# sbokov/AddingDisparityFiltering

Hardware: AMD Instinct MI355X
Metric: filtered Mpixels/s (+ achieved HBM GB/s) on 4K disparity, 1/2/4/8 GPUs vs CPU ref (higher is better)
Workload: dtype f32

## Files before the change

### addingdisparityfiltering_amd/_lib.py

```python
import ctypes as C
import os

_HERE = os.path.dirname(os.path.abspath(__file__))
LIB_PATH = os.environ.get("ADF_WLS_LIB") or os.path.join(_HERE, "libadf_wls.so")

ADF_OK, ADF_EBADARG, ADF_ESIZE, ADF_EHIP, ADF_ENOMEM, ADF_ENODEV = range(6)
SOLVER_EXACT, SOLVER_WAVE = 0, 1
PATH_CONF_BAND, PATH_FUSED_FIRST_PASS, PATH_MERGED_PREP, PATH_SCALED_FUSED, PATH_SCALED_HALF = 1, 2, 4, 8, 16
PATH_ROW_WEIGHTS_GUIDE = 32
HANDOFF_PAIR_PLANE, HANDOFF_IMAGE, HANDOFF_IMAGE_PAIR_TAIL = 0, 1, 2
DEPTH_8U, DEPTH_16S, DEPTH_32S, DEPTH_32F = 0, 3, 4, 5
SGBM_COST_BT, SGBM_COST_CENSUS_DENSE, SGBM_COST_CENSUS_SPARSE = 0, 1, 2
BM_COST_SAD, BM_COST_CENSUS_DENSE, BM_COST_CENSUS_SPARSE = 0, 1, 2
SGBM_COST_MCT_DENSE, SGBM_COST_MCT_SPARSE, SGBM_COST_CENSUS_CS = 4, 5, 6
BM_COST_MCT_DENSE, BM_COST_MCT_SPARSE, BM_COST_CENSUS_CS = 4, 5, 6
SGBM_RIGHT_MATCHER, SGBM_RIGHT_FROM_VOLUME = 0, 1
MISSING_NONE, MISSING_MIN, MISSING_VALUE = 0, 1, 2
WMF_EXP, WMF_IV1, WMF_IV2, WMF_COS, WMF_JAC, WMF_OFF = range(6)
WMF_WEIGHT_ONE, WMF_TABLE_LEVELS, WMF_MAX_RADIUS = 65536, 3 * 256 * 256, 31
GF_MAX_RADIUS = 31
DTF_NC, DTF_IC, DTF_RF, DT_MAX_ITERS = 0, 1, 2, 8
DT_NC_MAX_RADIUS = 127
JBF_MAX_RADIUS = 31
BORDER_REPLICATE, BORDER_REFLECT, BORDER_WRAP, BORDER_REFLECT_101 = 1, 2, 3, 4
# ... 52 lines not shown
    ("adf_wls_set_lambda", _i, [_vp, _d]),
    ("adf_wls_get_lambda", _i, [_vp, C.POINTER(_d)]),
    ("adf_wls_set_sigma_color", _i, [_vp, _d]),
    ("adf_wls_get_sigma_color", _i, [_vp, C.POINTER(_d)]),
    ("adf_wls_set_lrc_thresh", _i, [_vp, _i]),
    ("adf_wls_get_lrc_thresh", _i, [_vp, C.POINTER(_i)]),
    ("adf_wls_set_depth_discontinuity_radius", _i, [_vp, _i]),
    ("adf_wls_get_depth_discontinuity_radius", _i, [_vp, C.POINTER(_i)]),
    ("adf_wls_set_fgs_params", _i, [_vp, _d, _i]),
    ("adf_wls_set_solver", _i, [_vp, _i]),
    ("adf_wls_get_solver", _i, [_vp, C.POINTER(_i)]),
    ("adf_wls_get_last_solver", _i, [_vp, C.POINTER(_i)]),
    ("adf_wls_get_last_path", _i, [_vp, C.POINTER(_i)]),
    ("adf_wls_get_last_solver_path", _i, [_vp, C.POINTER(_i)]),
    ("adf_wls_get_last_handoff", _i, [_vp, C.POINTER(_i)]),
    ("adf_wls_filter_device", _i, _FILTER_DEV),
    ("adf_wls_filter_host", _i, _FILTER_DEV[:-1]),
    ("adf_wls_filter_scaled_device", _i, _FILTER_SCALED_DEV),
    ("adf_wls_filter_scaled_host", _i, _FILTER_SCALED_DEV[:-1]),
    ("adf_wls_filter_f32_device", _i, _FILTER_DEV),
    ("adf_wls_filter_f32_host", _i, _FILTER_DEV[:-1]),
    ("adf_wls_filter_scaled_f32_device", _i, _FILTER_SCALED_DEV),
    ("adf_wls_filter_scaled_f32_host", _i, _FILTER_SCALED_DEV[:-1]),
    ("adf_wls_filter_typed_device", _i, _FILTER_TYPED_DEV),
    ("adf_wls_filter_typed_host", _i, _FILTER_TYPED_DEV[:-1]),
    ("adf_wls_get_confidence_device", _i, [_vp, _i, _vp, _pd, _vp]),
    ("adf_wls_get_confidence_host", _i, [_vp, _i, _vp, _pd]),
    ("adf_wls_get_device", _i, [_vp, C.POINTER(_i)]),
    ("adf_wls_get_roi", _i, [_vp, C.POINTER(Rect)]),
    ("adf_wls_sync", _i, [_vp, _vp]),
# ... 124 lines not shown
```

### addingdisparityfiltering_amd/csrc/adf_api.hip

```cpp
#include "adf_host.h"

#include <cmath>
#include <cstdio>
#include <cstdlib>
#include <cstring>
#include <new>

using namespace adf;

static inline int round_up(int v, int m) { return (v + m - 1) / m * m; }
template <class T> static const T* pairs_on(const T* p, ptrdiff_t pair_stride, int k)
{
    return p ? (const T*)((const char*)p + (ptrdiff_t)k * pair_stride) : nullptr;
}

static Geom make_geom(int W, int H, int rx, int ry, int rw, int rh)
{
    Geom g;
    g.W = W; g.H = H; g.rx = rx; g.ry = ry; g.rw = rw; g.rh = rh;
    g.pw = round_up(rw, 64);
    g.ph = round_up(rh, 64);
    size_t a = (size_t)round_up(rh, TILE_ROWS) * g.pw, b = (size_t)rw * g.ph;
    g.plane = ((a > b ? a : b) + 63) / 64 * 64;
    g.frame = (size_t)W * H;
// ... 67 lines not shown
    int epilogue; void* out; ptrdiff_t stride, pair_stride; int x0, y0, cn, c;
};

static double epilogue_bytes(int epilogue)
{
    return (epilogue == EPI_F32 || epilogue == EPI_WLS_CONF_F32) ? 4.0 : epilogue == EPI_U8 ? 1.0 : 2.0;
}

template <class Args>
static void set_final_out(Args& a, const FinalOut& fo)
{
    a.out = fo.out; a.out_stride = fo.stride; a.out_pair_stride = fo.pair_stride;
    a.out_x0 = fo.x0; a.out_y0 = fo.y0; a.out_cn = fo.cn; a.out_c = fo.c;
}

static int run_passes(bool wave, const Geom& g, const SolvePlanes& p, int n_rhs, float lambda, float atten, int num_iter,
                      const FinalOut& fo, int n_pairs, hipStream_t st, Profiler* prof = nullptr,
                      const FusedInputs* fuse = nullptr, const GuideWeights* gw = nullptr, float* image = nullptr, int image_m = 0)
{
    const double px = (double)g.rw * g.rh * n_pairs;
    float lam = lambda;
    for (int it = 0; it < num_iter; it++, lam *= atten) {
        const bool fused = it == 0 && fuse, last = it == num_iter - 1;
        const int epi = last ? fo.epilogue : EPI_PLANES;
        const double lo_b = (fused && fuse->lo_conf) ? 6.0 * fuse->lo_scale_x * fuse->lo_scale_y : (fused && fuse->dl_f32) ? 8.0 : 6.0;
        const double wb = gw ? (double)gw->ch : 4.0;
        const double hb = fused ? (wb + lo_b + 8.0) * px : (wb + 8.0 * n_rhs) * px;
        const double out_b = (last ? epilogue_bytes(fo.epilogue) : 4.0 * n_rhs) * px;
        const double vb = (4.0 + 4.0 * n_rhs) * px + out_b;
        if (wave) {
            WavePassArgs h{}, v{};
            h.C = p.CH; h.U0 = p.A0; h.U1 = p.A1;
            h.nscan = g.rh; h.len = g.rw; h.pitch = g.pw; h.plane = g.plane; h.lambda = lam;
            if (fused) h.fuse = *fuse;
            if (gw) h.gw = *gw;
            v.C = p.CV; v.U0 = p.A0; v.U1 = p.A1;
            v.nscan = g.rw; v.len = g.rh; v.pitch = g.pw; v.plane = g.plane; v.lambda = lam;
            if (last) set_final_out(v, fo);
            if (image && last && it > 0) {
                h.image = v.image = image; h.image_m = v.image_m = image_m;
                h.image_plane = v.image_plane = wave_image_floats(g.pw, image_m);
            }
            {
                ProfScope ps(prof, fused ? K_PASS_H_FIRST : K_PASS_H, hb, hb, st);
                HIP_TRY(launch_wave_hpass(h, n_rhs, n_pairs, st));
            }
            ProfScope ps(prof, last ? K_PASS_V_LAST : K_PASS_V, vb, vb, st);
            HIP_TRY(launch_wave_vpass(v, n_rhs, epi, n_pairs, st));
        } else {
            PassArgs h{}, v{};
            h.C = p.CH; h.U0 = p.A0; h.U1 = p.A1; h.D = p.D; h.F0 = p.F0; h.F1 = p.F1; h.O0 = p.B0; h.O1 = p.B1;
            h.nscan = g.rh; h.len = g.rw; h.pitch_in = g.ph; h.pitch_out = g.pw; h.plane = g.plane; h.lambda = lam;
            v.C = p.CV; v.U0 = p.B0; v.U1 = p.B1; v.D = p.D; v.F0 = p.F0; v.F1 = p.F1; v.O0 = p.A0; v.O1 = p.A1;
            v.nscan = g.rw; v.len = g.rh; v.pitch_in = g.pw; v.pitch_out = g.ph; v.plane = g.plane; v.lambda = lam;
            if (last) set_final_out(v, fo);
            {
// ... 44 lines not shown
    DevBuf stage;
    DevBuf scaled;
    size_t ws_limit = (size_t)64 << 30;
    Profiler prof;
    long long ws_sig[8] = {0, 0, 0, 0, 0, 0, 0, 0};
    hipStream_t side = nullptr;
    hipEvent_t ev_fork = nullptr, ev_join = nullptr;
    bool overlap = true;
    struct LazyConf { bool pending = false; ConfResize resize{}; } lazy_conf;
    bool scaled_half = true;
    bool scaled_fuse = true;
    bool conf_band = true;
    bool merge_small = true;
    bool row_weights_guide = true;
    bool handoff_image = true;
    long long handoff_min_px = HANDOFF_IMAGE_MIN_PX;
    int last_handoff = ADF_HANDOFF_PAIR_PLANE;
    static bool null_caller_of(hipStream_t s) { return s == nullptr || s == hipStreamLegacy || s == hipStreamPerThread; }
    int ensure_side(hipStream_t caller)
    {
        if (side) return ADF_OK;
        int least = 0, greatest = 0, prio = 0, cp = 0;
        if (hipDeviceGetStreamPriorityRange(&least, &greatest) != hipSuccess) { least = greatest = 0; (void)hipGetLastError(); }
        if (null_caller_of(caller) || stream_is_capturing(caller) || hipStreamGetPriority(caller, &cp) != hipSuccess) { cp = 0; (void)hipGetLastError(); }
        prio = (cp != greatest) ? greatest : (greatest < least ? greatest + 1 : greatest);
        if (null_caller_of(caller)) HIP_TRY(hipStreamCreateWithFlags(&side, hipStreamNonBlocking));
        else HIP_TRY(hipStreamCreateWithPriority(&side, hipStreamNonBlocking, prio));
        HIP_TRY(hipEventCreateWithFlags(&ev_fork, hipEventDisableTiming));
        HIP_TRY(hipEventCreateWithFlags(&ev_join, hipEventDisableTiming));
        return ADF_OK;
    }
};
// ... 10 lines not shown
    if (!h) return fail(ADF_ENOMEM, "adf_wls_create: out of host memory");
    if (hipGetDevice(&h->device) != hipSuccess) { delete h; return fail(ADF_EHIP, "hipGetDevice failed"); }
    h->use_confidence = use_confidence != 0;
    h->left_offset = l; h->right_offset = r; h->top_offset = t; h->bottom_offset = b;
    h->min_disp = 0; (void)min_disp;
    if (const char* e = getenv("ADF_WS_LIMIT_GB")) {
        double gb = atof(e);
        if (gb > 0) h->ws_limit = (size_t)(gb * (double)((size_t)1 << 30));
    }
    if (const char* e = getenv("ADF_NO_OVERLAP")) h->overlap = atoi(e) == 0;
    if (const char* e = getenv("ADF_CONF_BAND")) h->conf_band = atoi(e) != 0;
    if (const char* e = getenv("ADF_SCALED_FUSE")) h->scaled_fuse = atoi(e) != 0;
    if (const char* e = getenv("ADF_ROW_WEIGHTS_GUIDE")) h->row_weights_guide = atoi(e) != 0;
    if (const char* e = getenv("ADF_LO_HALF")) h->scaled_half = atoi(e) != 0;
    if (const char* e = getenv("ADF_LAST_HANDOFF_IMAGE")) h->handoff_image = atoi(e) != 0;
    if (const char* e = getenv("ADF_LAST_HANDOFF_MIN_PX")) h->handoff_min_px = atoll(e);
    if (const char* e = getenv("ADF_MERGE_SMALL")) h->merge_small = atoi(e) != 0;
    *out = h;
    return ADF_OK;
}

extern "C" void adf_wls_destroy(adf_wls_t* h)
{
    if (!h) return;
    DeviceScope ds(h->device);
    h->lut.release(); h->ws.release(); h->conf.release(); h->stage.release(); h->scaled.release();
    h->prof.destroy();
    if (h->ev_fork) hipEventDestroy(h->ev_fork);
    if (h->ev_join) hipEventDestroy(h->ev_join);
    if (h->side) hipStreamDestroy(h->side);
// ... 18 lines not shown
    return ADF_OK;
}

extern "C" int adf_wls_set_solver(adf_wls_t* h, int solver)
{
    NEED_HANDLE(h);
    if (solver != ADF_SOLVER_EXACT && solver != ADF_SOLVER_WAVE) return fail(ADF_EBADARG, "unknown solver %d", solver);
    h->solver = solver;
    return ADF_OK;
}
extern "C" int adf_wls_get_solver(const adf_wls_t* h, int* v) { NEED_HANDLE(h); if (v) *v = h->solver; return ADF_OK; }
extern "C" int adf_wls_get_last_solver(const adf_wls_t* h, int* v) { NEED_HANDLE(h); if (v) *v = h->last_solver; return ADF_OK; }
extern "C" int adf_wls_get_last_path(const adf_wls_t* h, int* v) { NEED_HANDLE(h); if (v) *v = h->last_path; return ADF_OK; }
extern "C" int adf_wls_get_last_solver_path(const adf_wls_t* h, int* v) { NEED_HANDLE(h); if (v) *v = h->last_solver_path; return ADF_OK; }
extern "C" int adf_wls_get_last_handoff(const adf_wls_t* h, int* v) { NEED_HANDLE(h); if (v) *v = h->last_handoff; return ADF_OK; }

extern "C" int adf_wls_get_device(const adf_wls_t* h, int* device) { NEED_HANDLE(h); if (device) *device = h->device; return ADF_OK; }
extern "C" int adf_wls_get_roi(const adf_wls_t* h, adf_rect* roi) { NEED_HANDLE(h); if (roi) *roi = h->roi; return ADF_OK; }
extern "C" size_t adf_wls_workspace_bytes(const adf_wls_t* h)
{
    return h ? h->ws.bytes + h->conf.bytes + h->stage.bytes + h->scaled.bytes + h->lut.bytes() : 0;
}

extern "C" int adf_wls_sync(adf_wls_t* h, void* stream)
{
    NEED_HANDLE(h);
    DeviceScope ds(h->device);
    HIP_TRY(hipStreamSynchronize((hipStream_t)stream));
    return ADF_OK;
}
// ... 293 lines not shown
        HIP_TRY(launch_conf_left(ca, n, st));
        return ADF_OK;
    }
    const double fill = o.fill ? fill_bytes(F - P, false, o.fill->out_f32 ? 4.0 : 2.0).alg : 0.0;
    ProfScope ps(prof, K_LRC, lrc_bytes(F, P, o.U0 != nullptr, m.rhs_f32() ? 4.0 : 2.0, fill), st);
    HIP_TRY(launch_lrc_prologue(lrc_args(m, o, g, r), n, st));
    return ADF_OK;
}

struct ChunkPlan {
    ConfStage stage;
    bool fork_weights;
    bool outside_on_side;
    bool guide_rows;
    bool image;
};

struct WlsPlan {
    Geom g;
    bool wave;
    RhsSource rhs;
    bool band;
    bool quant_planes;
    Geom glo; bool lo_band; size_t dhi_bytes;
    size_t per_pair; int chunk;
    int image_m;
    bool image_in_chor;
    ChunkPlan full, tail;
    int path;
    int solver_path;
    bool fused_first() const { return rhs == RHS_FUSED_VIEW || rhs == RHS_FUSED_LO; }
};

static ChunkPlan plan_chunk(const adf_wls* h, ConfStage stage, bool wave, bool guide_rows, bool image)
{
    const bool fork = stage != CONF_NONE && stage != CONF_MERGED && h->overlap;
    return ChunkPlan{stage, fork, fork && wave && stage != CONF_TWO_KERNEL, guide_rows && stage != CONF_MERGED, image};
}

static GuideWeights guide_weights(const adf_wls* h, const uint8_t* guide, const View& v, const Geom& g)
{
    return GuideWeights{guide, v.stride, v.pair_stride, v.ch, g.rx, g.ry, h->lut.cur};
}

static WlsPlan plan_wls(const adf_wls* h, const WlsCall& c)
{
    WlsPlan p{};
    const bool conf = h->use_confidence, f32in = c.dm.f32;
    const View& v = c.view;
    const Geom g = p.g = make_geom(v.W, v.H, c.rhi.x, c.rhi.y, c.rhi.width, c.rhi.height);
    p.wave = h->solver == ADF_SOLVER_WAVE && wave_fits(g);
    MapSource m = caller_maps(c.dm);
// ... 29 lines not shown
    const int image_m = (conf && p.wave && h->handoff_image && h->num_iter >= 2 && wave_hpass_image_fits(g.rw)) ? wave_vpass_image_m(g.rh) : 0;
    const long long roi_px = (long long)g.rw * g.rh;
    const bool may_merge = p.band && h->merge_small && prep_small_fits(g, h->disc_radius, v.ch, 1) && prep_small_guide_fits(g, v.stride, v.ch);
    auto chunk_for = [&](int im) {
        p.image_m = im;
        p.image_in_chor = im && guide_rows && !may_merge;
        p.per_pair = wls_pair_ws_bytes(g, conf, p.wave, !p.band, p.quant_planes, im, p.image_in_chor);
        p.chunk = (int)(h->ws_limit / p.per_pair);
        if (p.chunk < 1) p.chunk = 1;
        if (p.chunk > c.n_pairs) p.chunk = c.n_pairs;
    };
    chunk_for(image_m);
    if (image_m && roi_px * p.chunk < h->handoff_min_px) chunk_for(0);
    auto chunk_of = [&](int n) {
        const bool merged = p.band && h->merge_small && prep_small_fits(g, h->disc_radius, v.ch, n) && prep_small_guide_fits(g, v.stride, v.ch);
        return plan_chunk(h, merged ? CONF_MERGED : stage, p.wave, guide_rows, p.image_m && roi_px * n >= h->handoff_min_px);
    };
    p.full = chunk_of(p.chunk);
    p.tail = chunk_of(c.n_pairs % p.chunk ? c.n_pairs % p.chunk : p.chunk);
    p.path = ((p.band || p.lo_band) ? ADF_PATH_CONF_BAND : 0) |
             (p.fused_first() ? ADF_PATH_FUSED_FIRST_PASS : 0) |
             ((p.full.stage == CONF_MERGED || p.tail.stage == CONF_MERGED) ? ADF_PATH_MERGED_PREP : 0);
    p.solver_path = (p.full.guide_rows || p.tail.guide_rows) ? ADF_PATH_ROW_WEIGHTS_GUIDE : 0;
    if (p.rhs == RHS_FUSED_LO)
        p.path |= ADF_PATH_SCALED_FUSED |
                  (wave_hpass_lo_half(first_pass_probe(lo_fuse(h, c, p.lo_band, UNALLOCATED, m, nullptr, g), g.rw)) ? ADF_PATH_SCALED_HALF : 0);
    return p;
}

struct ScaledBufs { char* dhi; float *cl, *cr, *clo; float* taps; };

static int scaled_buffers(adf_wls_t* h, const WlsCall& c, const WlsPlan& plan, hipStream_t st, ScaledBufs& b, MapSource& lo)
// ... 43 lines not shown
    const bool conf = h->use_confidence, wave = plan.wave;
    const Geom& g = plan.g;
    const View& vw = c.view;
    const OutMap& om = c.om;
    const adf_rect& roi = c.rhi;
    const int n_pairs = c.n_pairs, W = vw.W, H = vw.H, gch = vw.ch;
    const double ob_px = (double)om.esz(), db_px = (double)c.dm.esz();
    Profiler* prof = &h->prof;
    int rc;
    ScaledBufs sb{};
    MapSource lo{};
    if (c.scaled && (rc = scaled_buffers(h, c, plan, st, sb, lo))) return rc;
    h->roi = roi; h->last_W = W; h->last_H = H; h->last_pairs = n_pairs;
    h->last_cpitch = g.cpitch; h->last_cx0 = g.cx0; h->last_path = 0; h->last_solver_path = 0;
    h->last_solver = wave ? ADF_SOLVER_WAVE : ADF_SOLVER_EXACT;
    h->last_handoff = ADF_HANDOFF_PAIR_PLANE;
    if ((rc = h->ws.reserve(plan.per_pair * (size_t)plan.chunk, st, FILL_ZERO))) return rc;
    if (conf && !c.scaled && (rc = ensure_conf_planes(h, g, n_pairs, st))) return rc;
    {
        const long long sig[8] = {W, H, roi.x, roi.y, roi.width, roi.height,
                                  (long long)plan.image_in_chor * 1024 + (long long)plan.image_m * 16 + (long long)plan.quant_planes * 8 + (long long)plan.band * 4 + (long long)wave * 2 + conf, plan.chunk};
        if (memcmp(sig, h->ws_sig, sizeof(sig)) != 0) {
            HIP_TRY(hipMemsetAsync(h->ws.p, 0, h->ws.bytes, st));
            memcpy(h->ws_sig, sig, sizeof(sig));
        }
    }
    float* base = (float*)h->ws.p;
    auto take = [&](size_t elems) { float* p = base; base += elems * (size_t)plan.chunk; return p; };
    SolvePlanes p{};
    p.CH = take(g.plane);
    float* const image_rest = plan.image_in_chor ? take(wave_image_floats(g.pw, plan.image_m) - g.plane) : nullptr;
// ... 4 lines not shown
    if (conf) {
        p.A1 = take(g.plane);
        if (!wave) { p.F1 = take(g.plane); p.B1 = take(g.plane); }
    }
    float* const image = !plan.image_m ? nullptr : plan.image_in_chor ? p.CH : take(wave_image_floats(g.pw, plan.image_m));
    const size_t qframe = (size_t)quant_pitch(W) * H;
    int16_t* const qL = plan.quant_planes ? (int16_t*)take(qframe) : nullptr;
    int16_t* const qR = qL ? qL + qframe * (size_t)plan.chunk : nullptr;
    if (conf && !plan.band) { cL = take(g.frame); cR = take(g.frame); }
    const int orient_h = wave ? ORIENT_N : ORIENT_T;
    const int orient_u2 = wave ? ORIENT_PAIR : ORIENT_T;
    const int orient_cv = wave ? ORIENT_STRIP : ORIENT_N;
    const int16_t fill = (int16_t)(16 * (h->min_disp - 1));
    const ConfRule rule = conf_rule(h, c);
    h->last_path = plan.path; h->last_solver_path = plan.solver_path;
    h->last_handoff = (plan.full.image && plan.tail.image) ? ADF_HANDOFF_IMAGE : plan.full.image ? ADF_HANDOFF_IMAGE_PAIR_TAIL : ADF_HANDOFF_PAIR_PLANE;

    for (int first = 0; first < n_pairs; first += plan.chunk) {
        const int n = (n_pairs - first < plan.chunk) ? n_pairs - first : plan.chunk;
        const ChunkPlan& cp = n == plan.chunk ? plan.full : plan.tail;
        const uint8_t* gv = pairs_on(vw.p, vw.pair_stride, first);
        void* o = (char*)om.p + (ptrdiff_t)first * om.pair_stride;
        float* confp = conf ? (float*)h->conf.p + (size_t)first * g.cframe : nullptr;
        const double F = (double)g.frame * n, P = (double)g.rw * g.rh * n;
        MapSource m = c.scaled ? lo.from(first) : caller_maps(c.dm).from(first);
        OutsideArgs oa{o, om.stride, om.pair_stride, fill, om.f32 ? 1 : 0, c.scaled ? nullptr : confp, g};
        auto fill_outside = [&](hipStream_t s) {
            ProfScope ps(prof, K_FILL, fill_bytes(F - P, oa.conf != nullptr, ob_px), s);
            return launch_outside(oa, n, s);
        };
// ... 42 lines not shown
            ConfOut out{confp, cL, cR};
            if (plan.rhs == RHS_CONF_KERNEL) { out.U0 = p.A0; out.U1 = p.A1; out.orient = orient_u2; }
            if (cp.stage == CONF_TWO_KERNEL) out.fill = &oa;
            if ((rc = conf_stage(prof, cp.stage, m, g, rule, out, n, st))) return rc;
            if (cp.stage != CONF_TWO_KERNEL && !cp.outside_on_side) HIP_TRY(fill_outside(st));
            break;
        }
        }
        if (plan.rhs == RHS_PLAIN || plan.rhs == RHS_CONF_PROLOGUE) HIP_TRY(prologue(plan.rhs == RHS_CONF_PROLOGUE));
        if (cp.fork_weights) HIP_TRY(hipStreamWaitEvent(st, h->ev_join, 0));
        const FusedInputs fuse = plan.rhs == RHS_FUSED_LO
            ? lo_fuse(h, c, plan.lo_band, sb.clo + (size_t)first * c.dW * c.dH, m, sb.taps, g) : view_fuse(confp, m, g);
        const int epi = conf ? (om.f32 ? EPI_WLS_CONF_F32 : EPI_WLS_CONF) : (om.f32 ? EPI_F32 : EPI_I16);
        FinalOut fo{epi, o, om.stride, om.pair_stride, roi.x, roi.y, 1, 0};
        rc = run_passes(wave, g, p, conf ? 2 : 1, (float)h->lambda, (float)h->atten, h->num_iter, fo, n, st, prof,
                        plan.fused_first() ? &fuse : nullptr, cp.guide_rows ? &gw : nullptr, cp.image ? image : nullptr, plan.image_m);
        if (rc) return rc;
    }
    return ADF_OK;
}

static int wls_filter_device(adf_wls_t* h, int n_pairs, const DispMaps& dm, int dW, int dH, const View& view, const OutMap& om,
                             const adf_rect* roi, hipStream_t st)
{
    NEED_HANDLE(h);
    WlsCall c;
    int rc = check_call(h, n_pairs, dm, dW, dH, view, om, roi, c);
    if (rc) return rc;
    DeviceScope ds(h->device);
    h->lazy_conf.pending = false;
    if ((rc = h->lut.ensure((float)h->sigma_color, st))) return rc;
// ... 352 lines not shown
```

### addingdisparityfiltering_amd/csrc/adf_internal.h

```cpp
#pragma once

#include <hip/hip_runtime.h>
#include <stddef.h>
#include <stdint.h>
#include "../../include/adf_wls.h"

#define ADF_LUT_LEVELS (3 * 256 * 256)
#define ADF_EPS 1e-43f

namespace adf {

struct Geom {
    int W, H;
    int rx, ry, rw, rh;
    int pw, ph;
    size_t plane;
    size_t frame;
    int cpitch, cx0;
    size_t cframe;
};

enum Orient { ORIENT_N = 0, ORIENT_T = 1, ORIENT_PAIR = 2, ORIENT_STRIP = 3 };
#define ADF_STRIP 16
constexpr int TILE_ROWS = 2;
// ... 144 lines not shown
hipError_t launch_plain_prologue(const PlainPrologueArgs& a, int n_pairs, hipStream_t st);
hipError_t launch_quantise_maps(const QuantArgs& a, hipStream_t st);
hipError_t launch_weights(const WeightArgs& a, int n_pairs, hipStream_t st);
bool weights_stream_fits(const WeightArgs& a);
hipError_t launch_resize_linear(const ResizeArgs& a, int n_pairs, hipStream_t st);
hipError_t launch_exact_pass(const PassArgs& a, int n_rhs, int epilogue, int n_pairs, hipStream_t st);
hipError_t launch_wave_hpass(const WavePassArgs& a, int n_rhs, int n_pairs, hipStream_t st);
hipError_t launch_wave_vpass(const WavePassArgs& a, int n_rhs, int epilogue, int n_pairs, hipStream_t st);
int wave_max_row_len();
bool wave_hpass_can_fuse(const WavePassArgs& a);
bool wave_hpass_can_fuse_lo(const WavePassArgs& a);
bool wave_hpass_lo_half(const WavePassArgs& a);
bool wave_hpass_guide_fits(const WavePassArgs& a);
int wave_max_col_len();
bool wave_hpass_image_fits(int row_len);
int wave_vpass_image_m(int col_len);
inline size_t wave_image_floats(int pitch, int m) { return (size_t)pitch * (size_t)(64 * m) * 2; }
int max_disc_radius();

namespace tile {
constexpr int TX = 64;
constexpr int TY = 32;
constexpr int NT = 256;
}

#if defined(__HIPCC__)
__device__ __forceinline__ size_t pair_index(int i, int j, int pw)
{
    constexpr int TR = TILE_ROWS;
    return (size_t)(i / TR) * (size_t)(2 * TR * pw) + (size_t)((j >> 4) * (32 * TR) + (i % TR) * 32 + (j & 15));
// ... 69 lines not shown
```

### addingdisparityfiltering_amd/csrc/fgs_wave_h.hip

```cpp
#include "fgs_wave_common.h"
#include "prep_bodies.h"

#include <algorithm>

namespace adf {

namespace {
using namespace wave;

constexpr int H_TWO_WAVE_MAX = 60;

constexpr int FUSE_NONE = 0, FUSE_VIEW = 1, FUSE_LO = 2, FUSE_LO_HALF = 3, FUSE_VIEW_F32 = 4;
constexpr int WS_PLANE = 0, WS_GUIDE1 = 1, WS_GUIDE3 = 3;

typedef float v4f __attribute__((ext_vector_type(4)));

struct RowPos {
    int lane, wv;
    int v0;
    int nvec;
    int nvecU;
    size_t off;
    size_t offU;
};
// ... 625 lines not shown
        __syncthreads();
#pragma unroll
        for (int k = 0; k < MQ; k++) {
            const int idx = 64 * (k + half * MQ) + lane;
            if (idx < p.nvecU) store_nt(stage[64 * k + lane], d4 + ((unsigned)(idx >> 3) * strip_step + (unsigned)(idx & 7)));
        }
        __syncthreads();
    }
}

template <int M, int R, int FUSED, int NW = 1, int WS = WS_PLANE, bool IMAGE = false>
__global__ void __launch_bounds__(64 * NW, (M > (NW == 2 ? 40 : H_TWO_WAVE_MAX) && R > 1) ? 1 : 2) wave_hpass_kernel(WavePassArgs a)
{
    static_assert(M % 4 == 0 && M >= 4, "chunk length must be a multiple of 4");
    static_assert(NW == 1 || NW == 2, "one or two wavefronts per row");
    static_assert(!IMAGE || (R == 2 && FUSED == FUSE_NONE && NW == 1), "the last hand-off's image: a plain one-wave pass of two right-hand sides");
    constexpr bool LO = FUSED == FUSE_LO || FUSED == FUSE_LO_HALF;
    constexpr bool PAIR = R > 1;
    constexpr bool GUIDE = WS != WS_PLANE;
    static_assert(!GUIDE || (NW == 1 && !LO), "the guide forms: one-wave rows whose prologue leaves the staging buffer alone");
    __shared__ __attribute__((aligned(16))) float lut_head[GUIDE ? GW_HEAD : 1];
    __shared__ float4 stage_all[NW][LO ? lo_stage_vec4(M) : M * 16];
    __shared__ float xch[NW == 2 ? 5 : 1];
    __shared__ float red[NW == 2 ? 5 : 1][NW == 2 ? 128 : 1];
    __shared__ float xsol[NW == 2 ? 2 : 1][NW == 2 ? 128 : 1];
    const RowPos p = row_pos<M, PAIR, NW>(a);
    const int lane = p.lane, wv = p.wv;
    float4* stage = stage_all[wv];

    float4 tC[M / 4], t0[M / 4], t1[M / 4];
    GuideRaw<M, WS> tG;
// ... 55 lines not shown
        pcr64<R>(lane, al, be, ga, p0, p1, xs0, xs1);
        xL0 = __shfl_up(xs0, 1); xL1 = (R > 1) ? __shfl_up(xs1, 1) : 0.0f;
        if (lane == 0) { xL0 = 0.0f; xL1 = 0.0f; }
    }
    chunk_solve<M, R>(c, f0, f1, a_s, xL0, xL1, xs0, xs1);

    int lane_s = lane;
    asm volatile("" : "+v"(lane_s));
    if constexpr (IMAGE) store_image<M>(a, p, stage, lane_s, f0, f1);
    else if constexpr (PAIR) store_pair<M>(a, p, stage, lane_s, f0, f1);
    else store_plain<M>(a, p, stage, lane_s, f0);
}

constexpr bool lo_half_bucket(int m, int nw) { return !(m == 60 && nw == 1); }

constexpr bool guide_bucket(int nw) { return nw == 1; }

template <int M, int WS>
hipError_t launch_h_guide(const WavePassArgs& a, int n_rhs, dim3 grid, hipStream_t st)
{
    if (a.fuse.conf_in) {
        if (n_rhs != 2) return hipErrorInvalidValue;
        if (a.fuse.dl_f32) hipLaunchKernelGGL((wave_hpass_kernel<M, 2, FUSE_VIEW_F32, 1, WS>), grid, dim3(64), 0, st, a);
        else hipLaunchKernelGGL((wave_hpass_kernel<M, 2, FUSE_VIEW, 1, WS>), grid, dim3(64), 0, st, a);
    } else if (n_rhs == 2 && a.image) hipLaunchKernelGGL((wave_hpass_kernel<M, 2, FUSE_NONE, 1, WS, true>), grid, dim3(64), 0, st, a);
    else if (n_rhs == 2) hipLaunchKernelGGL((wave_hpass_kernel<M, 2, FUSE_NONE, 1, WS>), grid, dim3(64), 0, st, a);
    else hipLaunchKernelGGL((wave_hpass_kernel<M, 1, FUSE_NONE, 1, WS>), grid, dim3(64), 0, st, a);
    return hipGetLastError();
}

template <int M, int NW = 1>
hipError_t launch_h(const WavePassArgs& a, int n_rhs, int n_pairs, hipStream_t st)
{
    dim3 grid(a.nscan, n_pairs), block(64 * NW);
    if (a.gw.guide) {
        if constexpr (guide_bucket(NW)) {
            if (a.gw.ch == 1) return launch_h_guide<M, WS_GUIDE1>(a, n_rhs, grid, st);
            if (a.gw.ch == 3) return launch_h_guide<M, WS_GUIDE3>(a, n_rhs, grid, st);
        }
        return hipErrorInvalidValue;
    }
    if (a.fuse.lo_conf) {
        if (n_rhs != 2 || !a.fuse.lo_taps) return hipErrorInvalidValue;
        const int n = ((a.len + 3) / 4) * 4;
        hipLaunchKernelGGL(lo_tap_table_kernel, dim3((n + 255) / 256), dim3(256), 0, st, a.fuse.lo_taps, n, a.len, a.fuse.hi_x0, a.fuse.lo_scale_x, a.fuse.lo_w);
        bool half = false;
        if constexpr (lo_half_bucket(M, NW)) {
            half = wave_hpass_lo_half(a);
            if (half) hipLaunchKernelGGL((wave_hpass_kernel<M, 2, FUSE_LO_HALF, NW>), grid, block, 0, st, a);
        }
        if (!half) hipLaunchKernelGGL((wave_hpass_kernel<M, 2, FUSE_LO, NW>), grid, block, 0, st, a);
    } else if (a.fuse.conf_in) {
        if (n_rhs != 2) return hipErrorInvalidValue;
        if (a.fuse.dl_f32) hipLaunchKernelGGL((wave_hpass_kernel<M, 2, FUSE_VIEW_F32, NW>), grid, block, 0, st, a);
        else hipLaunchKernelGGL((wave_hpass_kernel<M, 2, FUSE_VIEW, NW>), grid, block, 0, st, a);
    } else if (n_rhs == 2 && a.image) {
        if constexpr (NW == 1) hipLaunchKernelGGL((wave_hpass_kernel<M, 2, FUSE_NONE, 1, WS_PLANE, true>), grid, block, 0, st, a);
        else return hipErrorInvalidValue;
    } else if (n_rhs == 2) hipLaunchKernelGGL((wave_hpass_kernel<M, 2, FUSE_NONE, NW>), grid, block, 0, st, a);
    else hipLaunchKernelGGL((wave_hpass_kernel<M, 1, FUSE_NONE, NW>), grid, block, 0, st, a);
    return hipGetLastError();
}

constexpr Bucket ROW_BUCKETS[] = {{4, 64}, {8, 64}, {16, 64}, {20, 64}, {28, 64}, {40, 64}, {56, 64}, {60, 64}, {64, 64},
                                  {40, 128}, {48, 128}, {56, 128}, {60, 128}, {64, 128}};
constexpr int N_ROW_BUCKETS = sizeof(ROW_BUCKETS) / sizeof(ROW_BUCKETS[0]);

void pick_row_bucket(int len, int& m, int& nw)
{
    const Bucket& b = ROW_BUCKETS[bucket_index(ROW_BUCKETS, len)];
// ... 19 lines not shown
    if (!a.gw.guide || !a.gw.lut || (a.gw.ch != 1 && a.gw.ch != 3) || a.fuse.lo_conf) return false;
    if ((reinterpret_cast<uintptr_t>(a.gw.lut) & 15u) != 0 || a.gw.x0 < 0 || a.gw.y0 < 0) return false;
    if (a.len < 2 || a.len > wave_max_row_len()) return false;
    int m, nw;
    pick_row_bucket(a.len, m, nw);
    return guide_bucket(nw);
}

bool wave_hpass_image_fits(int row_len)
{
    if (row_len < 2 || row_len > wave_max_row_len()) return false;
    int m, nw;
    pick_row_bucket(row_len, m, nw);
    return nw == 1;
}

bool wave_hpass_lo_half(const WavePassArgs& a)
{
    if (!(a.fuse.lo_conf && a.fuse.lo_half && a.fuse.lo_scale_x == 0.5 && (a.fuse.hi_x0 & 1) == 0 && a.fuse.hi_x0 >= 2)) return false;
    int m, nw;
    pick_row_bucket(a.len, m, nw);
    return lo_half_bucket(m, nw);
}

bool wave_hpass_can_fuse_lo(const WavePassArgs& a)
{
    if (!a.fuse.lo_conf || !a.fuse.lo_dl || a.fuse.lo_w < 2 || a.fuse.lo_w > 65535 || a.fuse.lo_h < 1 || a.len < 2 || a.len > wave_max_row_len()) return false;
    if ((reinterpret_cast<uintptr_t>(a.fuse.lo_conf) & 3u) != 0 || (reinterpret_cast<uintptr_t>(a.fuse.lo_dl) & 1u) != 0) return false;
    if (a.fuse.lo_dl_stride % 2 != 0 || a.fuse.lo_dl_pair % 2 != 0) return false;
    if (!(a.fuse.lo_scale_x > 0.0 && a.fuse.lo_scale_y > 0.0) || a.fuse.hi_x0 < 0 || a.fuse.hi_y0 < 0) return false;
// ... 7 lines not shown
            if (clast < cfirst) continue;
            int s_first, s_last; float f_;
            lin_tap(a.fuse.hi_x0 + cfirst, a.fuse.lo_scale_x, a.fuse.lo_w, s_first, f_);
            lin_tap(a.fuse.hi_x0 + clast, a.fuse.lo_scale_x, a.fuse.lo_w, s_last, f_);
            if (s_last + 2 - s_first > cap) return false;
        }
    return true;
}

hipError_t launch_wave_hpass(const WavePassArgs& a, int n_rhs, int n_pairs, hipStream_t st)
{
    if (a.len < 2 || a.len > wave_max_row_len() || a.pitch % 64 != 0 || a.pitch < a.len) return hipErrorInvalidValue;
    if (a.fuse.lo_conf && !wave_hpass_can_fuse_lo(a)) return hipErrorInvalidValue;
    if (!a.fuse.lo_conf && a.fuse.conf_in && !wave_hpass_can_fuse(a)) return hipErrorInvalidValue;
    if (a.gw.guide && !wave_hpass_guide_fits(a)) return hipErrorInvalidValue;
    if (a.image && (n_rhs != 2 || a.fuse.conf_in || a.fuse.lo_conf || !wave_hpass_image_fits(a.len) || a.image_m < 1 ||
                    a.nscan > 64 * a.image_m || a.image_plane < wave_image_floats(a.pitch, a.image_m)))
        return hipErrorInvalidValue;
    return dispatch_index<N_ROW_BUCKETS>(bucket_index(ROW_BUCKETS, a.len), [&](auto I) {
        constexpr Bucket b = ROW_BUCKETS[decltype(I)::value];
        return launch_h<b.m, b.chunks / 64>(a, n_rhs, n_pairs, st);
    });
}

}
```

### addingdisparityfiltering_amd/csrc/fgs_wave_v.hip

```cpp
#include "fgs_wave_common.h"

namespace adf {

namespace {
using namespace wave;

constexpr int VT = 512;
constexpr int VC = 16;
typedef float v4f __attribute__((ext_vector_type(4)));

template <int EPI>
__device__ __forceinline__ v2f epi_value(v2f u0, v2f u1)
{
    if (EPI == EPI_WLS_CONF || EPI == EPI_WLS_CONF_F32) {
        const v2f sc = vsplat(0x1p64f);
        return u0 * (vrcp_nr(vfma(u1, sc, vsplat(ADF_EPS * 0x1p64f))) * sc);
    }
    return u0;
}

template <int EPI>
__device__ __forceinline__ unsigned epi_pack16(v2f u0, v2f u1)
{
    const v2f x = epi_value<EPI>(u0, u1);
// ... 49 lines not shown
    }
}

template <int R>
__device__ __forceinline__ unsigned vstep(int r0, int i, int pitch)
{
    constexpr unsigned TR = TILE_ROWS;
    if (R > 1) return ((((unsigned)r0 + (unsigned)i + 1u) & (TR - 1u)) == 0u) ? 2u * TR * (unsigned)pitch * 4u - (TR - 1u) * 128u : 128u;
    return (unsigned)pitch * 4u;
}

template <int M, int R, int EPI, int VCW = VC, int NCH = 64, bool IMG = false>
__global__ void __launch_bounds__(VT) wave_vpass_kernel(WavePassArgs a)
{
    static_assert((VCW == 16 && NCH == 64) || (VCW == 8 && NCH == 128), "whole strips of 64 chunks or half strips of 128");
    static_assert(!IMG || (R == 2 && VCW == VC && (EPI == EPI_WLS_CONF || EPI == EPI_WLS_CONF_F32)), "the image: whole strips, both right-hand sides, the filter's epilogues");
    static_assert((VCW / 2) * NCH == VT, "one thread per (chunk, column pair)");
    constexpr int XPN = VCW / 2;
    __shared__ float nb[4][NCH][VCW];
    __shared__ float red[5][VCW][NCH];
    __shared__ float xs[2][VCW][NCH];
    const int tid = threadIdx.x;
    const int xp = tid & (XPN - 1), cidx = tid / XPN;
    int strip = VCW == VC ? (int)blockIdx.x : (int)(blockIdx.x >> 1);
    if (VCW == VC) {
        const int nfull = (int)(gridDim.x / 32) * 32;
        if ((EPI != EPI_PLANES || R == 1) && (int)blockIdx.x < nfull) {
            const int grp = blockIdx.x >> 5, w = blockIdx.x & 31;
            strip = (grp << 5) + ((w & 7) << 2) + (w >> 3);
        }
    }
// ... 149 lines not shown
        }
    }
}

template <int M, int VCW = VC, int NCH = 64>
hipError_t launch_v(const WavePassArgs& a, int n_rhs, int epi, int n_pairs, hipStream_t st)
{
    dim3 grid(a.pitch / VCW, n_pairs), block(VT);
    constexpr int N_EPI = N_EPILOGUES;
    if (n_rhs < 1 || n_rhs > 2 || epi < 0 || epi >= N_EPI) return hipErrorInvalidValue;
    return dispatch_index<2 * N_EPI>((n_rhs - 1) * N_EPI + epi, [&](auto K) {
        constexpr int R = decltype(K)::value / N_EPI + 1, EPI = decltype(K)::value % N_EPI;
        if constexpr (R == 1 && (EPI == EPI_WLS_CONF || EPI == EPI_WLS_CONF_F32)) return hipErrorInvalidValue;
        else {
            if (a.image) {
                if constexpr (R == 2 && VCW == VC && (EPI == EPI_WLS_CONF || EPI == EPI_WLS_CONF_F32)) {
                    if (a.image_m != M || a.image_plane < wave_image_floats(a.pitch, M)) return hipErrorInvalidValue;
                    hipLaunchKernelGGL((wave_vpass_kernel<M, R, EPI, VCW, NCH, true>), grid, block, 0, st, a);
                    return hipGetLastError();
                } else return hipErrorInvalidValue;
            }
            hipLaunchKernelGGL((wave_vpass_kernel<M, R, EPI, VCW, NCH>), grid, block, 0, st, a);
            return hipGetLastError();
        }
    });
}

constexpr Bucket COL_BUCKETS[] = {{2, 64}, {4, 64}, {8, 64}, {12, 64}, {18, 64}, {26, 64}, {34, 64}, {20, 128}, {26, 128}, {34, 128}};
constexpr int N_COL_BUCKETS = sizeof(COL_BUCKETS) / sizeof(COL_BUCKETS[0]);

}
// ... 22 lines not shown
```

### addingdisparityfiltering_amd/ximgproc.py

```python
import ctypes as C
import functools
import math

import numpy as np

from . import _lib
from ._lib import SGBM_COST_BT, SGBM_COST_CENSUS_DENSE, SGBM_COST_CENSUS_SPARSE
from ._lib import BM_COST_SAD, BM_COST_CENSUS_DENSE, BM_COST_CENSUS_SPARSE
from ._lib import SGBM_COST_MCT_DENSE, SGBM_COST_MCT_SPARSE, SGBM_COST_CENSUS_CS
from ._lib import BM_COST_MCT_DENSE, BM_COST_MCT_SPARSE, BM_COST_CENSUS_CS
from ._lib import SGBM_RIGHT_MATCHER, SGBM_RIGHT_FROM_VOLUME
from ._lib import WMF_EXP, WMF_IV1, WMF_IV2, WMF_COS, WMF_JAC, WMF_OFF
from ._lib import GF_MAX_RADIUS
from ._lib import DTF_NC, DTF_IC, DTF_RF, DT_MAX_ITERS, DT_NC_MAX_RADIUS
from ._lib import RGF_MAX_ITERS
from ._lib import JBF_MAX_RADIUS, BORDER_REPLICATE, BORDER_REFLECT, BORDER_WRAP, BORDER_REFLECT_101
from ._lib import AdfError, HANDOFF_IMAGE, HANDOFF_IMAGE_PAIR_TAIL, HANDOFF_PAIR_PLANE, PATH_CONF_BAND, PATH_FUSED_FIRST_PASS, PATH_MERGED_PREP, PATH_ROW_WEIGHTS_GUIDE, PATH_SCALED_FUSED, PATH_SCALED_HALF, Rect, SOLVER_EXACT, SOLVER_WAVE

try:
    import torch
except Exception:
    torch = None


# ... 177 lines not shown

    def getSolver(self):
        return _read(_lib.lib().adf_wls_get_solver, C.c_int, self._h)

    def getLastSolver(self):
        return _read(_lib.lib().adf_wls_get_last_solver, C.c_int, self._h)

    def getLastPath(self):
        return _read(_lib.lib().adf_wls_get_last_path, C.c_int, self._h)

    def getLastSolverPath(self):
        return _read(_lib.lib().adf_wls_get_last_solver_path, C.c_int, self._h)

    def getLastHandoff(self):
        return _read(_lib.lib().adf_wls_get_last_handoff, C.c_int, self._h)

    def enableProfiling(self, on=True):
        _lib.check(_lib.lib().adf_wls_profile_enable(self._h, int(bool(on))))

    def readProfile(self):
        buf = (_lib.KernelTime * 16)()
        n = C.c_int()
        _lib.check(_lib.lib().adf_wls_profile_read(self._h, buf, 16, C.byref(n)))
        return {buf[k].name.decode(): dict(launches=buf[k].launches, total_ms=buf[k].total_ms,
                                           alg_bytes=buf[k].alg_bytes, moved_bytes=buf[k].moved_bytes)
                for k in range(n.value)}

    def workspaceBytes(self):
        return int(_lib.lib().adf_wls_workspace_bytes(self._h))

# ... 1242 lines not shown
```

### include/adf_wls.h

```cpp
#ifndef ADF_WLS_H
#define ADF_WLS_H

#include <stddef.h>
#include <stdint.h>

#ifdef __cplusplus
extern "C" {
#endif

#define ADF_VERSION 100

enum adf_status {
    ADF_OK = 0,
    ADF_EBADARG = 1,
    ADF_ESIZE = 2,
    ADF_EHIP = 3,
    ADF_ENOMEM = 4,
    ADF_ENODEV = 5
};

enum adf_solver { ADF_SOLVER_EXACT = 0, ADF_SOLVER_WAVE = 1 };

enum adf_depth { ADF_8U = 0, ADF_16S = 3, ADF_32S = 4, ADF_32F = 5 };

// ... 25 lines not shown
int adf_wls_set_solver(adf_wls_t* h, int solver);
int adf_wls_get_solver(const adf_wls_t* h, int* solver);
int adf_wls_get_last_solver(const adf_wls_t* h, int* solver);
#define ADF_PATH_CONF_BAND 1
#define ADF_PATH_FUSED_FIRST_PASS 2
#define ADF_PATH_MERGED_PREP 4
#define ADF_PATH_SCALED_FUSED 8
#define ADF_PATH_SCALED_HALF 16
int adf_wls_get_last_path(const adf_wls_t* h, int* path_flags);
#define ADF_PATH_ROW_WEIGHTS_GUIDE 32
int adf_wls_get_last_solver_path(const adf_wls_t* h, int* path_flags);
#define ADF_HANDOFF_PAIR_PLANE 0
#define ADF_HANDOFF_IMAGE 1
#define ADF_HANDOFF_IMAGE_PAIR_TAIL 2
int adf_wls_get_last_handoff(const adf_wls_t* h, int* form);

int adf_wls_filter_device(adf_wls_t* h, int n_pairs,
                          const int16_t* disp_left, ptrdiff_t disp_left_stride, ptrdiff_t disp_left_pair_stride,
                          const uint8_t* left_view, ptrdiff_t view_stride, ptrdiff_t view_pair_stride,
                          int view_channels, int W, int H,
                          int16_t* out, ptrdiff_t out_stride, ptrdiff_t out_pair_stride,
                          const int16_t* disp_right, ptrdiff_t disp_right_stride, ptrdiff_t disp_right_pair_stride,
                          const adf_rect* roi, void* stream);

int adf_wls_filter_host(adf_wls_t* h, int n_pairs,
                        const int16_t* disp_left, ptrdiff_t disp_left_stride, ptrdiff_t disp_left_pair_stride,
                        const uint8_t* left_view, ptrdiff_t view_stride, ptrdiff_t view_pair_stride,
                        int view_channels, int W, int H,
                        int16_t* out, ptrdiff_t out_stride, ptrdiff_t out_pair_stride,
                        const int16_t* disp_right, ptrdiff_t disp_right_stride, ptrdiff_t disp_right_pair_stride,
// ... 412 lines not shown
```

Baseline: 42870.

## Extend image hand-off between wave passes to inner and first iterations

The image-layout hand-off between the horizontal and vertical wave passes, previously used only on the last iteration, now also runs on the inner iterations. On the first iteration it runs when the fused int16 view prologue is used. The goal is to avoid the pair-plane round trip through HBM on every iteration, not just the final one. It adds new kernel template instantiations (the fused-view horizontal pass with an image, and the plain-plane vertical pass with an image), an env toggle, and a query API for how many inner hand-offs happened. The risk is extra register or LDS pressure in those variants and more dispatch paths that can reject unsupported shapes.

```diff
diff --git a/addingdisparityfiltering_amd/_lib.py b/addingdisparityfiltering_amd/_lib.py
--- a/addingdisparityfiltering_amd/_lib.py
+++ b/addingdisparityfiltering_amd/_lib.py
@@ -90,6 +90,7 @@
     ("adf_wls_get_last_path", _i, [_vp, C.POINTER(_i)]),
     ("adf_wls_get_last_solver_path", _i, [_vp, C.POINTER(_i)]),
     ("adf_wls_get_last_handoff", _i, [_vp, C.POINTER(_i)]),
+    ("adf_wls_get_inner_handoffs", _i, [_vp, C.POINTER(_i), C.POINTER(_i)]),
     ("adf_wls_filter_device", _i, _FILTER_DEV),
     ("adf_wls_filter_host", _i, _FILTER_DEV[:-1]),
     ("adf_wls_filter_scaled_device", _i, _FILTER_SCALED_DEV),
diff --git a/addingdisparityfiltering_amd/csrc/adf_api.hip b/addingdisparityfiltering_amd/csrc/adf_api.hip
--- a/addingdisparityfiltering_amd/csrc/adf_api.hip
+++ b/addingdisparityfiltering_amd/csrc/adf_api.hip
@@ -105,9 +105,24 @@
     a.out_x0 = fo.x0; a.out_y0 = fo.y0; a.out_cn = fo.cn; a.out_c = fo.c;
 }
 
+struct HandoffImage {
+    float* image = nullptr; int m = 0; bool inner = false, first = false;
+    bool at(int it, int num_iter) const
+    {
+        if (!image || num_iter < 2) return false;
+        return it == num_iter - 1 ? true : it > 0 ? inner : first;
+    }
+    int inner_count(int num_iter) const
+    {
+        int n = 0;
+        for (int it = 0; it + 1 < num_iter; it++) n += at(it, num_iter);
+        return n;
+    }
+};
+
 static int run_passes(bool wave, const Geom& g, const SolvePlanes& p, int n_rhs, float lambda, float atten, int num_iter,
                       const FinalOut& fo, int n_pairs, hipStream_t st, Profiler* prof = nullptr,
-                      const FusedInputs* fuse = nullptr, const GuideWeights* gw = nullptr, float* image = nullptr, int image_m = 0)
+                      const FusedInputs* fuse = nullptr, const GuideWeights* gw = nullptr, const HandoffImage& ho = HandoffImage{})
 {
     const double px = (double)g.rw * g.rh * n_pairs;
     float lam = lambda;
@@ -128,9 +143,9 @@
             v.C = p.CV; v.U0 = p.A0; v.U1 = p.A1;
             v.nscan = g.rw; v.len = g.rh; v.pitch = g.pw; v.plane = g.plane; v.lambda = lam;
             if (last) set_final_out(v, fo);
-            if (image && last && it > 0) {
-                h.image = v.image = image; h.image_m = v.image_m = image_m;
-                h.image_plane = v.image_plane = wave_image_floats(g.pw, image_m);
+            if (ho.at(it, num_iter)) {
+                h.image = v.image = ho.image; h.image_m = v.image_m = ho.m;
+                h.image_plane = v.image_plane = wave_image_floats(g.pw, ho.m);
             }
             {
                 ProfScope ps(prof, fused ? K_PASS_H_FIRST : K_PASS_H, hb, hb, st);
@@ -205,8 +220,10 @@
     bool merge_small = true;
     bool row_weights_guide = true;
     bool handoff_image = true;
+    bool handoff_inner = true;
     long long handoff_min_px = HANDOFF_IMAGE_MIN_PX;
     int last_handoff = ADF_HANDOFF_PAIR_PLANE;
+    int last_inner[2] = {0, 0};
     static bool null_caller_of(hipStream_t s) { return s == nullptr || s == hipStreamLegacy || s == hipStreamPerThread; }
     int ensure_side(hipStream_t caller)
     {
@@ -247,6 +264,7 @@
     if (const char* e = getenv("ADF_ROW_WEIGHTS_GUIDE")) h->row_weights_guide = atoi(e) != 0;
     if (const char* e = getenv("ADF_LO_HALF")) h->scaled_half = atoi(e) != 0;
     if (const char* e = getenv("ADF_LAST_HANDOFF_IMAGE")) h->handoff_image = atoi(e) != 0;
+    if (const char* e = getenv("ADF_INNER_HANDOFF_IMAGE")) h->handoff_inner = atoi(e) != 0;
     if (const char* e = getenv("ADF_LAST_HANDOFF_MIN_PX")) h->handoff_min_px = atoll(e);
     if (const char* e = getenv("ADF_MERGE_SMALL")) h->merge_small = atoi(e) != 0;
     *out = h;
@@ -295,6 +313,14 @@
 extern "C" int adf_wls_get_last_path(const adf_wls_t* h, int* v) { NEED_HANDLE(h); if (v) *v = h->last_path; return ADF_OK; }
 extern "C" int adf_wls_get_last_solver_path(const adf_wls_t* h, int* v) { NEED_HANDLE(h); if (v) *v = h->last_solver_path; return ADF_OK; }
 extern "C" int adf_wls_get_last_handoff(const adf_wls_t* h, int* v) { NEED_HANDLE(h); if (v) *v = h->last_handoff; return ADF_OK; }
+
+extern "C" int adf_wls_get_inner_handoffs(const adf_wls_t* h, int* full, int* tail)
+{
+    NEED_HANDLE(h);
+    if (full) *full = h->last_inner[0];
+    if (tail) *tail = h->last_inner[1];
+    return ADF_OK;
+}
 
 extern "C" int adf_wls_get_device(const adf_wls_t* h, int* device) { NEED_HANDLE(h); if (device) *device = h->device; return ADF_OK; }
 extern "C" int adf_wls_get_roi(const adf_wls_t* h, adf_rect* roi) { NEED_HANDLE(h); if (roi) *roi = h->roi; return ADF_OK; }
@@ -618,6 +644,7 @@
     bool outside_on_side;
     bool guide_rows;
     bool image;
+    bool inner_image;
 };
 
 struct WlsPlan {
@@ -630,16 +657,17 @@
     size_t per_pair; int chunk;
     int image_m;
     bool image_in_chor;
+    bool first_image;
     ChunkPlan full, tail;
     int path;
     int solver_path;
     bool fused_first() const { return rhs == RHS_FUSED_VIEW || rhs == RHS_FUSED_LO; }
 };
 
-static ChunkPlan plan_chunk(const adf_wls* h, ConfStage stage, bool wave, bool guide_rows, bool image)
+static ChunkPlan plan_chunk(const adf_wls* h, ConfStage stage, bool wave, bool guide_rows, bool image, bool inner_image)
 {
     const bool fork = stage != CONF_NONE && stage != CONF_MERGED && h->overlap;
-    return ChunkPlan{stage, fork, fork && wave && stage != CONF_TWO_KERNEL, guide_rows && stage != CONF_MERGED, image};
+    return ChunkPlan{stage, fork, fork && wave && stage != CONF_TWO_KERNEL, guide_rows && stage != CONF_MERGED, image, image && inner_image};
 }
 
 static GuideWeights guide_weights(const adf_wls* h, const uint8_t* guide, const View& v, const Geom& g)
@@ -699,8 +727,9 @@
     if (image_m && roi_px * p.chunk < h->handoff_min_px) chunk_for(0);
     auto chunk_of = [&](int n) {
         const bool merged = p.band && h->merge_small && prep_small_fits(g, h->disc_radius, v.ch, n) && prep_small_guide_fits(g, v.stride, v.ch);
-        return plan_chunk(h, merged ? CONF_MERGED : stage, p.wave, guide_rows, p.image_m && roi_px * n >= h->handoff_min_px);
+        return plan_chunk(h, merged ? CONF_MERGED : stage, p.wave, guide_rows, p.image_m && roi_px * n >= h->handoff_min_px, h->handoff_inner);
     };
+    p.first_image = p.rhs == RHS_FUSED_VIEW && wave_hpass_first_image(view_fuse(planes, m, g));
     p.full = chunk_of(p.chunk);
     p.tail = chunk_of(c.n_pairs % p.chunk ? c.n_pairs % p.chunk : p.chunk);
     p.path = ((p.band || p.lo_band) ? ADF_PATH_CONF_BAND : 0) |
@@ -774,7 +803,7 @@
     h->roi = roi; h->last_W = W; h->last_H = H; h->last_pairs = n_pairs;
     h->last_cpitch = g.cpitch; h->last_cx0 = g.cx0; h->last_path = 0; h->last_solver_path = 0;
     h->last_solver = wave ? ADF_SOLVER_WAVE : ADF_SOLVER_EXACT;
-    h->last_handoff = ADF_HANDOFF_PAIR_PLANE;
+    h->last_handoff = ADF_HANDOFF_PAIR_PLANE; h->last_inner[0] = h->last_inner[1] = 0;
     if ((rc = h->ws.reserve(plan.per_pair * (size_t)plan.chunk, st, FILL_ZERO))) return rc;
     if (conf && !c.scaled && (rc = ensure_conf_planes(h, g, n_pairs, st))) return rc;
     {
@@ -809,6 +838,8 @@
     const int16_t fill = (int16_t)(16 * (h->min_disp - 1));
     const ConfRule rule = conf_rule(h, c);
     h->last_path = plan.path; h->last_solver_path = plan.solver_path;
+    auto handoff_of = [&](const ChunkPlan& cp) { return HandoffImage{cp.image ? image : nullptr, plan.image_m, cp.inner_image, cp.inner_image && plan.first_image}; };
+    if (wave) { h->last_inner[0] = handoff_of(plan.full).inner_count(h->num_iter); h->last_inner[1] = handoff_of(plan.tail).inner_count(h->num_iter); }
     h->last_handoff = (plan.full.image && plan.tail.image) ? ADF_HANDOFF_IMAGE : plan.full.image ? ADF_HANDOFF_IMAGE_PAIR_TAIL : ADF_HANDOFF_PAIR_PLANE;
 
     for (int first = 0; first < n_pairs; first += plan.chunk) {
@@ -881,7 +912,7 @@
         const int epi = conf ? (om.f32 ? EPI_WLS_CONF_F32 : EPI_WLS_CONF) : (om.f32 ? EPI_F32 : EPI_I16);
         FinalOut fo{epi, o, om.stride, om.pair_stride, roi.x, roi.y, 1, 0};
         rc = run_passes(wave, g, p, conf ? 2 : 1, (float)h->lambda, (float)h->atten, h->num_iter, fo, n, st, prof,
-                        plan.fused_first() ? &fuse : nullptr, cp.guide_rows ? &gw : nullptr, cp.image ? image : nullptr, plan.image_m);
+                        plan.fused_first() ? &fuse : nullptr, cp.guide_rows ? &gw : nullptr, handoff_of(cp));
         if (rc) return rc;
     }
     return ADF_OK;
diff --git a/addingdisparityfiltering_amd/csrc/adf_internal.h b/addingdisparityfiltering_amd/csrc/adf_internal.h
--- a/addingdisparityfiltering_amd/csrc/adf_internal.h
+++ b/addingdisparityfiltering_amd/csrc/adf_internal.h
@@ -182,6 +182,7 @@
 bool wave_hpass_guide_fits(const WavePassArgs& a);
 int wave_max_col_len();
 bool wave_hpass_image_fits(int row_len);
+bool wave_hpass_first_image(const FusedInputs& f);
 int wave_vpass_image_m(int col_len);
 inline size_t wave_image_floats(int pitch, int m) { return (size_t)pitch * (size_t)(64 * m) * 2; }
 int max_disc_radius();
diff --git a/addingdisparityfiltering_amd/csrc/fgs_wave_h.hip b/addingdisparityfiltering_amd/csrc/fgs_wave_h.hip
--- a/addingdisparityfiltering_amd/csrc/fgs_wave_h.hip
+++ b/addingdisparityfiltering_amd/csrc/fgs_wave_h.hip
@@ -663,7 +663,8 @@
 {
     static_assert(M % 4 == 0 && M >= 4, "chunk length must be a multiple of 4");
     static_assert(NW == 1 || NW == 2, "one or two wavefronts per row");
-    static_assert(!IMAGE || (R == 2 && FUSED == FUSE_NONE && NW == 1), "the last hand-off's image: a plain one-wave pass of two right-hand sides");
+    static_assert(!IMAGE || (R == 2 && (FUSED == FUSE_NONE || FUSED == FUSE_VIEW) && NW == 1),
+                  "a hand-off's image: a one-wave pass of two right-hand sides, plain or with the view-resolution int16 prologue");
     constexpr bool LO = FUSED == FUSE_LO || FUSED == FUSE_LO_HALF;
     constexpr bool PAIR = R > 1;
     constexpr bool GUIDE = WS != WS_PLANE;
@@ -749,6 +750,8 @@
 
 constexpr bool lo_half_bucket(int m, int nw) { return !(m == 60 && nw == 1); }
 
+constexpr bool FIRST_IMAGE = true;
+
 constexpr bool guide_bucket(int nw) { return nw == 1; }
 
 template <int M, int WS>
@@ -757,7 +760,10 @@
     if (a.fuse.conf_in) {
         if (n_rhs != 2) return hipErrorInvalidValue;
         if (a.fuse.dl_f32) hipLaunchKernelGGL((wave_hpass_kernel<M, 2, FUSE_VIEW_F32, 1, WS>), grid, dim3(64), 0, st, a);
-        else hipLaunchKernelGGL((wave_hpass_kernel<M, 2, FUSE_VIEW, 1, WS>), grid, dim3(64), 0, st, a);
+        else if (a.image) {
+            if constexpr (FIRST_IMAGE) hipLaunchKernelGGL((wave_hpass_kernel<M, 2, FUSE_VIEW, 1, WS, true>), grid, dim3(64), 0, st, a);
+            else return hipErrorInvalidValue;
+        } else hipLaunchKernelGGL((wave_hpass_kernel<M, 2, FUSE_VIEW, 1, WS>), grid, dim3(64), 0, st, a);
     } else if (n_rhs == 2 && a.image) hipLaunchKernelGGL((wave_hpass_kernel<M, 2, FUSE_NONE, 1, WS, true>), grid, dim3(64), 0, st, a);
     else if (n_rhs == 2) hipLaunchKernelGGL((wave_hpass_kernel<M, 2, FUSE_NONE, 1, WS>), grid, dim3(64), 0, st, a);
     else hipLaunchKernelGGL((wave_hpass_kernel<M, 1, FUSE_NONE, 1, WS>), grid, dim3(64), 0, st, a);
@@ -788,7 +794,10 @@
     } else if (a.fuse.conf_in) {
         if (n_rhs != 2) return hipErrorInvalidValue;
         if (a.fuse.dl_f32) hipLaunchKernelGGL((wave_hpass_kernel<M, 2, FUSE_VIEW_F32, NW>), grid, block, 0, st, a);
-        else hipLaunchKernelGGL((wave_hpass_kernel<M, 2, FUSE_VIEW, NW>), grid, block, 0, st, a);
+        else if (a.image) {
+            if constexpr (FIRST_IMAGE && NW == 1) hipLaunchKernelGGL((wave_hpass_kernel<M, 2, FUSE_VIEW, 1, WS_PLANE, true>), grid, block, 0, st, a);
+            else return hipErrorInvalidValue;
+        } else hipLaunchKernelGGL((wave_hpass_kernel<M, 2, FUSE_VIEW, NW>), grid, block, 0, st, a);
     } else if (n_rhs == 2 && a.image) {
         if constexpr (NW == 1) hipLaunchKernelGGL((wave_hpass_kernel<M, 2, FUSE_NONE, 1, WS_PLANE, true>), grid, block, 0, st, a);
         else return hipErrorInvalidValue;
@@ -838,6 +847,8 @@
     pick_row_bucket(row_len, m, nw);
     return nw == 1;
 }
+
+bool wave_hpass_first_image(const FusedInputs& f) { return FIRST_IMAGE && f.conf_in && !f.lo_conf && !f.dl_f32; }
 
 bool wave_hpass_lo_half(const WavePassArgs& a)
 {
@@ -875,7 +886,7 @@
     if (a.fuse.lo_conf && !wave_hpass_can_fuse_lo(a)) return hipErrorInvalidValue;
     if (!a.fuse.lo_conf && a.fuse.conf_in && !wave_hpass_can_fuse(a)) return hipErrorInvalidValue;
     if (a.gw.guide && !wave_hpass_guide_fits(a)) return hipErrorInvalidValue;
-    if (a.image && (n_rhs != 2 || a.fuse.conf_in || a.fuse.lo_conf || !wave_hpass_image_fits(a.len) || a.image_m < 1 ||
+    if (a.image && (n_rhs != 2 || a.fuse.lo_conf || (a.fuse.conf_in && (a.fuse.dl_f32 || !FIRST_IMAGE)) || !wave_hpass_image_fits(a.len) || a.image_m < 1 ||
                     a.nscan > 64 * a.image_m || a.image_plane < wave_image_floats(a.pitch, a.image_m)))
         return hipErrorInvalidValue;
     return dispatch_index<N_ROW_BUCKETS>(bucket_index(ROW_BUCKETS, a.len), [&](auto I) {
diff --git a/addingdisparityfiltering_amd/csrc/fgs_wave_v.hip b/addingdisparityfiltering_amd/csrc/fgs_wave_v.hip
--- a/addingdisparityfiltering_amd/csrc/fgs_wave_v.hip
+++ b/addingdisparityfiltering_amd/csrc/fgs_wave_v.hip
@@ -87,7 +87,7 @@
 __global__ void __launch_bounds__(VT) wave_vpass_kernel(WavePassArgs a)
 {
     static_assert((VCW == 16 && NCH == 64) || (VCW == 8 && NCH == 128), "whole strips of 64 chunks or half strips of 128");
-    static_assert(!IMG || (R == 2 && VCW == VC && (EPI == EPI_WLS_CONF || EPI == EPI_WLS_CONF_F32)), "the image: whole strips, both right-hand sides, the filter's epilogues");
+    static_assert(!IMG || (R == 2 && VCW == VC && (EPI == EPI_PLANES || EPI == EPI_WLS_CONF || EPI == EPI_WLS_CONF_F32)), "the image: whole strips, both right-hand sides, the plain pass or the filter's epilogues");
     static_assert((VCW / 2) * NCH == VT, "one thread per (chunk, column pair)");
     constexpr int XPN = VCW / 2;
     __shared__ float nb[4][NCH][VCW];
@@ -267,7 +267,7 @@
         if constexpr (R == 1 && (EPI == EPI_WLS_CONF || EPI == EPI_WLS_CONF_F32)) return hipErrorInvalidValue;
         else {
             if (a.image) {
-                if constexpr (R == 2 && VCW == VC && (EPI == EPI_WLS_CONF || EPI == EPI_WLS_CONF_F32)) {
+                if constexpr (R == 2 && VCW == VC && (EPI == EPI_PLANES || EPI == EPI_WLS_CONF || EPI == EPI_WLS_CONF_F32)) {
                     if (a.image_m != M || a.image_plane < wave_image_floats(a.pitch, M)) return hipErrorInvalidValue;
                     hipLaunchKernelGGL((wave_vpass_kernel<M, R, EPI, VCW, NCH, true>), grid, block, 0, st, a);
                     return hipGetLastError();
diff --git a/addingdisparityfiltering_amd/ximgproc.py b/addingdisparityfiltering_amd/ximgproc.py
--- a/addingdisparityfiltering_amd/ximgproc.py
+++ b/addingdisparityfiltering_amd/ximgproc.py
@@ -215,6 +215,11 @@
 
     def getLastHandoff(self):
         return _read(_lib.lib().adf_wls_get_last_handoff, C.c_int, self._h)
+
+    def getInnerHandoffs(self):
+        full, tail = C.c_int(0), C.c_int(0)
+        _lib.check(_lib.lib().adf_wls_get_inner_handoffs(self._h, C.byref(full), C.byref(tail)))
+        return full.value, tail.value
 
     def enableProfiling(self, on=True):
         _lib.check(_lib.lib().adf_wls_profile_enable(self._h, int(bool(on))))
diff --git a/include/adf_wls.h b/include/adf_wls.h
--- a/include/adf_wls.h
+++ b/include/adf_wls.h
@@ -63,6 +63,7 @@
 #define ADF_HANDOFF_IMAGE 1
 #define ADF_HANDOFF_IMAGE_PAIR_TAIL 2
 int adf_wls_get_last_handoff(const adf_wls_t* h, int* form);
+int adf_wls_get_inner_handoffs(const adf_wls_t* h, int* full, int* tail);
 
 int adf_wls_filter_device(adf_wls_t* h, int n_pairs,
                           const int16_t* disp_left, ptrdiff_t disp_left_stride, ptrdiff_t disp_left_pair_stride,
```

Measured after the change: 43920 (median of 6 runs). 2.5% higher.
